# CarloSaccardi/GAN-Leaks

Hardware: AMD Instinct MI355X
Metric: attack query-images/sec (10k queries x 100k samples) + AUROC delta vs ref (higher is better)
Workload: dtype split-f16 (hi+lo, f32 accumulate; generator) + i8->i32 exact (distance)

## Files before the change

### gan-leaks_amd/csrc/gl_conv.h

```cpp
#pragma once
#include "gl_common.h"

struct GlGatherConv {
    const float *in;
    unsigned in_bytes;
    int64_t positions;
    int H, W, Cin;
    int up;
    const float *wpack;
    int cols;
    int cols_pad;
    int ntaps;
    uint32_t tap_dy[4], tap_dx[4];
    float *out;
    int Ho, Wo, omul;
    int oy[4], ox[4];
    int planar;
    int64_t ld_planar;
    int out_mode;
    int *sat_flag;
    const float *scale, *shift;
    int cmod;
    int act;
    const float *residual;
    const float *zero;
    const void *tail_w;
    float *tail_out;
    int64_t tail_ld;
    float tail_scale;
    float pixnorm_act;
    const float *rgb_w, *rgb_b;
    float *rgb_out;
    int rgb_n;
    float rgb_inv_act;
    char *tap_V;
    const float *tap_coef;
    int64_t tap_ldv, tap_off;
    int64_t tap_row0;
    int tap_fmt;
    char *tap_pool;
    float tap_scale, tap_eps;
};

static inline bool gl_vrow_blocked(int64_t K1_halves) { return K1_halves * 2 >= (2ll << 20); }
static inline int64_t gl_vrow_capacity(int64_t n, int64_t K1_halves) { return gl_vrow_blocked(K1_halves) ? (n + 255) / 256 * 256 : n; }

#if defined(__HIPCC__)
__device__ __forceinline__ char *gl_vrow_elem(char *V, int64_t ldv, int64_t row, int64_t k)
{
    if (ldv >= 0) return V + row * ldv + k * 2;
    return V + ((row >> 8) * (-ldv) + (k >> 6)) * 32768 + (row & 255) * 128 + (k & 63) * 2;
}

__device__ __forceinline__ float gl_tap_value(float v, float inv, float coef)
{
    float x = v * inv;
    asm volatile("" : "+v"(x));
    float t = x * coef;
    asm volatile("" : "+v"(t));
    return t;
}
#endif

void gl_pack_tail_weights_host(const float *w48xC, int channels, float scale, void *out);

static inline int64_t gl_conv_k_index(int tap, int ci, int ntaps) { return ((int64_t)(ci / 32) * ntaps + tap) * 32 + (ci % 32); }

int gl_launch_gather_conv(gl_ctx *ctx, const GlGatherConv &p, int phases);

int gl_launch_gather_conv_h3(gl_ctx *ctx, const GlGatherConv &p, int phases);
int gl_conv_h3_tile_channels(const GlGatherConv &p, int phases);
bool gl_conv_h3_tap_fusable(const GlGatherConv &p, int phases);
bool gl_conv_halo_applies(const GlGatherConv &p, int phases);
int gl_launch_conv_halo_h3(gl_ctx *ctx, const GlGatherConv &p);
int gl_launch_split_rows(gl_ctx *ctx, const float *in, int64_t n, int d, int dpad, float scale, void *out);
void gl_split_weights_host(const float *w, size_t rows, size_t K, float scale, void *out);

int gl_launch_col2im_rgb_tanh(gl_ctx *ctx, const float *P, int64_t ldp, int64_t n_img, int H, int W, const float *bias, float *out_f32,
                              uint8_t *out_u8);
```

### gan-leaks_amd/csrc/gl_conv_h3.hip

```cpp
#include "gl_conv.h"
#include "gl_conv_h3_epi.h"
#include <cstdlib>
#include <type_traits>

namespace {

using gl_h3::v8h;
using gl_h3::v4h;
using gl_h3::v4f;

constexpr int HBK_BYTES = 128;

template <int WC, int WP, int TC = 4, int TP = 4, bool FUSE_TAIL = false, bool UP = false, bool T4 = false>
__global__ void __launch_bounds__(64 * WC * WP, 2) gather_conv_h3_kernel(const GlGatherConv p, int m_tiles, int n_tiles, int phases)
{
#if __HIP_DEVICE_COMPILE__
    constexpr int HTC = 16 * TC * WC, HTP = 16 * TP * WP;
    constexpr int W_BYTES = HTC * HBK_BYTES, X_BYTES = HTP * HBK_BYTES, BUF = W_BYTES + X_BYTES;
    constexpr int NW = WC * WP;
    constexpr int PW = (HTC / 8) / NW, PX = (HTP / 8) / NW;
    static_assert(!T4 || (HTP == 256 && TP == 4 && WP == 4 && PX == 4 && !UP && !FUSE_TAIL), "T4: the 256-position tile with 4 position-waves of 4 fragments");
    extern __shared__ __attribute__((aligned(16))) char smem[];

    const unsigned inner = (unsigned)phases * (unsigned)n_tiles;
    const unsigned id = gl_xcd_remap(blockIdx.x, (unsigned)m_tiles * inner);
    const int mt = (int)(id / inner);
    const int phase = (int)((id % inner) / (unsigned)n_tiles);
    const int nt = (int)(id % (unsigned)n_tiles);
    const int64_t m0 = (int64_t)mt * HTP;
    const int c0 = nt * HTC;

    const int tid0 = threadIdx.x, lane0 = tid0 & 63;
    const int wave = __builtin_amdgcn_readfirstlane(tid0 >> 6);
    const int wc = wave / WP, wp_ = wave % WP;

    const int K = p.ntaps * p.Cin;
    const int nk = K / 32;
    const int HW = p.H * p.W;
    const uint32_t tdy = p.tap_dy[phase], tdx = p.tap_dx[phase];
    const char *wbase = reinterpret_cast<const char *>(p.wpack) + (int64_t)phase * p.cols_pad * K * 4;

    const int rsub = lane0 >> 3, slot = lane0 & 7;
    constexpr int up = UP ? 1 : 0;
    const int Ws = p.W >> up, Hs = p.H >> up;
    constexpr unsigned kOOB = 0xC0000000u;
    const unsigned lead_bytes = (unsigned)(p.W + 1) * (unsigned)p.Cin * 4u;
    const __amdgpu_buffer_rsrc_t x_rsrc =
        __builtin_amdgcn_make_buffer_rsrc(const_cast<char *>(reinterpret_cast<const char *>(p.in)) - (up ? 0 : (int64_t)lead_bytes), 0,
                                          (int)(p.in_bytes + (up ? 0u : 2u * lead_bytes)), 0x00020000);
    const __amdgpu_buffer_rsrc_t w_rsrc = __builtin_amdgcn_make_buffer_rsrc(const_cast<char *>(wbase), 0, (int)((unsigned)p.cols_pad * (unsigned)K * 4u), 0x00020000);
    unsigned x_voff0 = kOOB, x_mask2[(PX + 1) / 2], w_voff0 = 0;
#pragma unroll
    for (int i = 0; i < (PX + 1) / 2; ++i) x_mask2[i] = 0;
    auto x_mask_of = [&](int i) -> unsigned { return (x_mask2[i >> 1] >> ((i & 1) * 16)) & 0xFFFFu; };
    int x_img[UP ? PX : 1], x_yx[UP ? PX : 1];
    {
        const int r = wave * PW * 8 + rsub;
        w_voff0 = ((unsigned)(c0 + r) * (unsigned)K) * 4u + (unsigned)(slot ^ rsub) * 16u;
    }
    const unsigned w_step = 8u * (unsigned)K * 4u, x_step = 8u * (unsigned)p.Cin * 4u;
    auto t4_pos = [](int r) -> int { const int f = r >> 4, wpp = f >> 2, j = f & 3; return (r & 15) * 16 + 4 * j + ((j + wpp) & 3); };
#pragma unroll
    for (int i = 0; i < PX; ++i) {
        const int r = (wave * PX + i) * 8 + rsub;
        const int chunk = slot ^ (r & 7);
        const int64_t pos = m0 + (T4 ? t4_pos(r) : r);
        if constexpr (UP) { x_img[i] = 0; x_yx[i] = 0; }
        if (pos < p.positions) {
            const int64_t img = pos / HW;
            const int rem = (int)(pos - img * HW);
            const int y = rem / p.W, x = rem - y * p.W;
            for (int t = 0; t < p.ntaps; ++t) {
                const int yy = y + (int)((tdy >> (2 * t)) & 3u) - 1, xx = x + (int)((tdx >> (2 * t)) & 3u) - 1;
                if ((yy >= 0) & (yy < p.H) & (xx >= 0) & (xx < p.W)) x_mask2[i >> 1] |= 1u << (t + (i & 1) * 16);
            }
            if (i == 0 || T4) { if (i == 0) x_voff0 = (unsigned)pos * (unsigned)p.Cin * 4u + (unsigned)chunk * 16u; }
            if constexpr (UP) { x_img[i] = (int)(img * Hs * Ws); x_yx[i] = y | (x << 16); }
        }
    }

    auto stage = [&](int kt, char *buf) {
        const int tap = kt % p.ntaps;
        const int cc = kt / p.ntaps;
        const int dy = (int)((tdy >> (2 * tap)) & 3u) - 1;
        const int dx = (int)((tdx >> (2 * tap)) & 3u) - 1;
        const unsigned tapbit = 1u << tap;
#pragma unroll
        for (int i = 0; i < PW; ++i)
            __builtin_amdgcn_raw_ptr_buffer_load_lds(w_rsrc, (gl_lptr)(buf + (wave * PW + i) * 1024), 16, w_voff0, (unsigned)kt * 128u + (unsigned)i * w_step, 0, 0);
        if (!up) {
            const unsigned soff = (unsigned)(((dy + 1) * p.W + (dx + 1)) * p.Cin) * 4u + (unsigned)cc * 128u;
#pragma unroll
            for (int i = 0; i < PX; ++i) {
                const unsigned voff = (x_mask_of(i) & tapbit) ? x_voff0 : kOOB;
                unsigned piece = (unsigned)i * x_step;
                if constexpr (T4) piece = (unsigned)(t4_pos((wave * PX + i) * 8) - t4_pos(wave * PX * 8)) * (unsigned)p.Cin * 4u;
                __builtin_amdgcn_raw_ptr_buffer_load_lds(x_rsrc, (gl_lptr)(buf + W_BYTES + (wave * PX + i) * 1024), 16, voff, soff + piece, 0, 0);
            }
        } else {
            const unsigned soff = (unsigned)cc * 128u;
#pragma unroll
            for (int i = 0; i < PX; ++i) {
                const int r = (wave * PX + i) * 8 + rsub;
                const int yy = (x_yx[UP ? i : 0] & 0xFFFF) + dy, xx = (x_yx[UP ? i : 0] >> 16) + dx;
                const unsigned pix = (unsigned)(x_img[UP ? i : 0] + (yy >> 1) * Ws + (xx >> 1));
                const unsigned voff = (x_mask_of(i) & tapbit) ? pix * (unsigned)p.Cin * 4u + (unsigned)((slot ^ (r & 7)) * 16) : kOOB;
                __builtin_amdgcn_raw_ptr_buffer_load_lds(x_rsrc, (gl_lptr)(buf + W_BYTES + (wave * PX + i) * 1024), 16, voff, soff, 0, 0);
            }
        }
    };

    v4f acc[TC][TP];
#pragma unroll
    for (int i = 0; i < TC; ++i)
#pragma unroll
        for (int j = 0; j < TP; ++j) acc[i][j] = (v4f){0.f, 0.f, 0.f, 0.f};

    const int frow0 = lane0 & 15, fk0 = lane0 >> 4;
    auto compute = [&](const char *cur, int kt) {
        const char *lw = cur + (wc * 16 * TC) * HBK_BYTES;
        const char *lx = cur + W_BYTES + (wp_ * 16 * TP) * HBK_BYTES;
        v8h w_hi[TC], w_lo[TC], x_hi[TP], x_lo[TP];
        unsigned skip = 0;
        if constexpr (T4) {
            const int tap = kt % p.ntaps;
            const int dy = (int)((tdy >> (2 * tap)) & 3u) - 1, dx = (int)((tdx >> (2 * tap)) & 3u) - 1;
#pragma unroll
            for (int j = 0; j < TP; ++j) {
                const int yy = j + dy, xx = ((j + wp_) & 3) + dx;
                skip |= ((yy < 0) | (yy > 3) | (xx < 0) | (xx > 3)) ? 1u << j : 0u;
            }
        }
#pragma unroll
        for (int i = 0; i < TC; ++i) {
            const int r = i * 16 + frow0;
            w_hi[i] = *reinterpret_cast<const v8h *>(lw + r * HBK_BYTES + ((fk0 ^ (r & 7)) << 4));
            w_lo[i] = *reinterpret_cast<const v8h *>(lw + r * HBK_BYTES + (((4 + fk0) ^ (r & 7)) << 4));
        }
#pragma unroll
        for (int j = 0; j < TP; ++j) {
            const int r = j * 16 + frow0;
            x_hi[j] = *reinterpret_cast<const v8h *>(lx + r * HBK_BYTES + ((fk0 ^ (r & 7)) << 4));
            x_lo[j] = *reinterpret_cast<const v8h *>(lx + r * HBK_BYTES + (((4 + fk0) ^ (r & 7)) << 4));
        }
        if constexpr (T4) {
#pragma unroll
            for (int j = 0; j < TP; ++j) {
                if ((skip >> j) & 1u) continue;
#pragma unroll
                for (int i = 0; i < TC; ++i) {
                    acc[i][j] = __builtin_amdgcn_mfma_f32_16x16x32_f16(w_lo[i], x_hi[j], acc[i][j], 0, 0, 0);
                    acc[i][j] = __builtin_amdgcn_mfma_f32_16x16x32_f16(w_hi[i], x_lo[j], acc[i][j], 0, 0, 0);
                    acc[i][j] = __builtin_amdgcn_mfma_f32_16x16x32_f16(w_hi[i], x_hi[j], acc[i][j], 0, 0, 0);
                }
            }
        } else {
#pragma unroll
            for (int i = 0; i < TC; ++i)
#pragma unroll
                for (int j = 0; j < TP; ++j) {
                    acc[i][j] = __builtin_amdgcn_mfma_f32_16x16x32_f16(w_lo[i], x_hi[j], acc[i][j], 0, 0, 0);
                    acc[i][j] = __builtin_amdgcn_mfma_f32_16x16x32_f16(w_hi[i], x_lo[j], acc[i][j], 0, 0, 0);
                    acc[i][j] = __builtin_amdgcn_mfma_f32_16x16x32_f16(w_hi[i], x_hi[j], acc[i][j], 0, 0, 0);
                }
        }
    };
    stage(0, smem);
    for (int kt = 0; kt < nk; ++kt) {
        __syncthreads();
        if (kt + 1 < nk) stage(kt + 1, smem + ((kt + 1) & 1) * BUF);
        compute(smem + (kt & 1) * BUF, kt);
    }

    __syncthreads();
    int tid_again = threadIdx.x;
    asm volatile("" : "+v"(tid_again));
    const int tid = tid_again, lane = tid_again & 63, frow = tid_again & 15, fk = (tid_again & 63) >> 4;
    int *orow = reinterpret_cast<int *>(smem);
    if (tid < HTP) {
        const int64_t pos = m0 + (T4 ? t4_pos(tid) : tid);
        int o = -1;
        if (pos < p.positions) {
            const int64_t img = pos / HW;
            const int rem = (int)(pos - img * HW);
            const int y = rem / p.W, x = rem - y * p.W;
            o = (int)((img * p.Ho + (y * p.omul + p.oy[phase])) * p.Wo + (x * p.omul + p.ox[phase]));
        }
        orow[tid] = o;
    }
    __syncthreads();
    int o4[TP];
#pragma unroll
    for (int j = 0; j < TP; ++j) o4[j] = orow[wp_ * 16 * TP + j * 16 + frow];
    const float relu_floor = p.act == 1 ? 0.0f : -__builtin_inff();
    const float neg_slope = p.act == 2 ? 0.2f : 1.0f;
    bool saturated = false;
    if constexpr (FUSE_TAIL) {
        static_assert((WC == 2 || WC == 1) && TC == 4 && TP == 4, "fused tail: waves of 64 channels x 64 positions, 64 or 128 channels in all");
        v8h b_hi[2][TP], b_lo[2][TP];
#pragma unroll
        for (int i = 0; i < TC; ++i) {
            const int ch = wc * 64 + i * 16 + 4 * fk;
            float sc[4], sh[4];
#pragma unroll
            for (int r = 0; r < 4; ++r) { sc[r] = p.scale[ch + r]; sh[r] = p.shift[ch + r]; }
#pragma unroll
            for (int j = 0; j < TP; ++j)
#pragma unroll
                for (int r = 0; r < 4; ++r) {
                    float t = fmaf(acc[i][j][r], sc[r], sh[r]);
                    t = fmaxf(fmaxf(t, t * neg_slope), relu_floor);
                    const float c = fminf(fmaxf(t, -65504.0f), 65504.0f);
                    saturated |= (c != t) && (o4[j] >= 0);
                    const _Float16 h = (_Float16)c;
                    b_hi[i >> 1][j][(i & 1) * 4 + r] = h;
                    b_lo[i >> 1][j][(i & 1) * 4 + r] = (_Float16)(c - (float)h);
                }
        }
        v4f pacc[3][TP];
#pragma unroll
        for (int pt = 0; pt < 3; ++pt)
#pragma unroll
            for (int j = 0; j < TP; ++j) pacc[pt][j] = (v4f){0.f, 0.f, 0.f, 0.f};
        const v8h *tw = reinterpret_cast<const v8h *>(p.tail_w) + (size_t)wc * 3 * 2 * 2 * 64;
#pragma unroll
        for (int pt = 0; pt < 3; ++pt)
#pragma unroll
            for (int s2 = 0; s2 < 2; ++s2) {
                const v8h a_hi = tw[((pt * 2 + s2) * 2 + 0) * 64 + frow * 4 + fk];
                const v8h a_lo = tw[((pt * 2 + s2) * 2 + 1) * 64 + frow * 4 + fk];
#pragma unroll
                for (int j = 0; j < TP; ++j) {
                    pacc[pt][j] = __builtin_amdgcn_mfma_f32_16x16x32_f16(a_lo, b_hi[s2][j], pacc[pt][j], 0, 0, 0);
                    pacc[pt][j] = __builtin_amdgcn_mfma_f32_16x16x32_f16(a_hi, b_lo[s2][j], pacc[pt][j], 0, 0, 0);
                    pacc[pt][j] = __builtin_amdgcn_mfma_f32_16x16x32_f16(a_hi, b_hi[s2][j], pacc[pt][j], 0, 0, 0);
                }
            }
        float *xch = reinterpret_cast<float *>(smem + 4096) + (size_t)wp_ * 3 * TP * 4 * 64;
        if (WC == 2 && wc == 1) {
#pragma unroll
            for (int pt = 0; pt < 3; ++pt)
#pragma unroll
                for (int j = 0; j < TP; ++j)
#pragma unroll
                    for (int r = 0; r < 4; ++r) xch[((pt * TP + j) * 4 + r) * 64 + lane] = pacc[pt][j][r];
        }
        if (WC == 2) __syncthreads();
        if (wc == 0) {
#pragma unroll
            for (int pt = 0; pt < 3; ++pt)
#pragma unroll
                for (int j = 0; j < TP; ++j) {
                    const int o = o4[j];
                    if (o < 0) continue;
#pragma unroll
                    for (int r = 0; r < 4; ++r) {
                        const float v = pacc[pt][j][r] + (WC == 2 ? xch[((pt * TP + j) * 4 + r) * 64 + lane] : 0.0f);
                        p.tail_out[(int64_t)(pt * 16 + 4 * fk + r) * p.tail_ld + o] = v * p.tail_scale;
                    }
                }
        }
    } else {
        saturated |= gl_h3::epilogue<WC, WP, TC, TP>(p, acc, c0, wc, wp_, lane, o4, smem, p.tap_V ? (p.Wo >> 4) : 0);
    }
    if (__any(saturated) && lane == 0) atomicAdd(p.sat_flag, 1);
#endif
}

__global__ void __launch_bounds__(256) split_rows_kernel(const float *__restrict__ in, int64_t n, int d, int dpad, float scale, char *__restrict__ out)
{
    const int64_t i = (int64_t)blockIdx.x * blockDim.x + threadIdx.x;
    if (i >= n * dpad) return;
    const int64_t r = i / dpad;
    const int c = (int)(i - r * dpad);
    const float v = c < d ? fminf(fmaxf(in[r * d + c] * scale, -65504.0f), 65504.0f) : 0.0f;
    const _Float16 hi = (_Float16)v;
    const _Float16 lo = (_Float16)(v - (float)hi);
    char *dst = out + (r * dpad + (c >> 5) * 32) * 4 + (c & 31) * 2;
    *reinterpret_cast<_Float16 *>(dst) = hi;
    *reinterpret_cast<_Float16 *>(dst + 64) = lo;
}

}

template <int WC, int WP, int TC = 4, int TP = 4, bool FUSE_TAIL = false, bool UP = false, bool T4 = false>
static int launch_h3(gl_ctx *ctx, const GlGatherConv &p, int phases)
{
    if constexpr (!UP && !FUSE_TAIL && !T4) {
        if (p.up) return launch_h3<WC, WP, TC, TP, FUSE_TAIL, true>(ctx, p, phases);
    }
    if constexpr (WC == 2 && WP == 4 && TC == 8 && TP == 4 && !UP && !FUSE_TAIL && !T4) {
        const bool plain = !p.up && !p.tail_w && !p.tap_V && !p.rgb_out && p.pixnorm_act == 0.0f && !p.planar;
        if (plain && p.H == 4 && p.W == 4 && gl_tuning_int("GL_H3_T4", 1)) return launch_h3<WC, WP, TC, TP, false, false, true>(ctx, p, phases);
    }
    constexpr int HTC = 16 * TC * WC, HTP = 16 * TP * WP;
    const int64_t m_tiles = gl_ceil_div(p.positions, HTP);
    const int n_tiles = (int)gl_ceil_div(p.cols, HTC);
    GL_REQUIRE(m_tiles * n_tiles * phases < (1ll << 31), "gather_conv_h3: grid too large");
    constexpr int lds = 2 * (HTC + HTP) * HBK_BYTES;
    auto kern = gather_conv_h3_kernel<WC, WP, TC, TP, FUSE_TAIL, UP, T4>;
    GL_ONCE_PER_DEVICE(ctx, \
        GL_HIP(hipFuncSetAttribute(reinterpret_cast<const void *>(kern), hipFuncAttributeMaxDynamicSharedMemorySize, lds)););
    gl_prof_scope prof_(ctx, GL_PROF_GATHER_CONV);
    hipLaunchKernelGGL(kern, dim3((unsigned)(m_tiles * n_tiles * phases)), dim3(64 * WC * WP), lds, ctx->stream, p, (int)m_tiles, n_tiles, phases);
    GL_LAUNCH_CHECK();
    return GL_OK;
}

static int h3_tile_choice(const GlGatherConv &p, int phases)
{
    if (p.tail_w) return p.cols == 128 ? 3 : 4;
    if (p.cols <= 64) return 1;
    if (p.cols % 256 == 0 && gl_ceil_div(p.positions, 256) * (p.cols / 256) * phases >= 256) return 2;
    const int wide128 = gl_tuning_int("GL_H3_TILE128", 1);
    if (wide128 && p.cols <= 128 && gl_ceil_div(p.positions, 512) * phases >= 512) return 5;
    return 0;
}

int gl_conv_h3_tile_channels(const GlGatherConv &p, int phases)
{
    if (gl_conv_halo_applies(p, phases)) return p.cols <= 64 ? 64 : 128;
    const int t = h3_tile_choice(p, phases);
    return (t == 2 || t == 5) ? 0 : (t == 1 || t == 4) ? 64 : 128;
}

bool gl_conv_h3_tap_fusable(const GlGatherConv &p, int phases)
{
    const int enabled = gl_tuning_int("GL_TAP_FUSE", 1);
    if (!enabled || phases != 1 || p.tail_w || p.out_mode != 2 || p.omul != 1 || p.Ho != p.H || p.Wo != p.W || p.planar) return false;
    if (p.cols > gl_conv_h3_tile_channels(p, phases) || p.H % 2 != 0 || p.W % 16 != 0) return false;
    if (gl_conv_halo_applies(p, phases)) return true;
    return (p.W == 16 || p.W == 32) && p.positions % 64 == 0;
}

int gl_launch_gather_conv_h3(gl_ctx *ctx, const GlGatherConv &p_in, int phases)
{
    gl_make_current(ctx);
    GlGatherConv p = p_in;
    p.sat_flag = ctx->h3_sat;
    GL_REQUIRE(p.Cin % 32 == 0, "gather_conv_h3: Cin=%d must be a multiple of 32", p.Cin);
    GL_REQUIRE(p.cmod > 0 && p.cmod % 4 == 0, "gather_conv_h3: cmod=%d must be a positive multiple of 4", p.cmod);
    GL_REQUIRE(p.cols_pad % 128 == 0 && p.cols <= p.cols_pad && p.cols % 4 == 0, "gather_conv_h3: cols=%d / cols_pad=%d (multiple of 128)", p.cols, p.cols_pad);
    GL_REQUIRE(phases >= 1 && phases <= 4 && p.ntaps >= 1 && p.ntaps <= 16, "gather_conv_h3: bad phases/taps");
    GL_REQUIRE(p.act >= 0 && p.act <= 2 && !p.residual, "gather_conv_h3: activation %d / residual not supported", p.act);
    GL_REQUIRE(p.out_mode != 2 || p.cols % 32 == 0, "gather_conv_h3: split output needs cols %% 32 == 0");
    GL_REQUIRE(p.up == 0 || (p.up == 1 && p.H % 2 == 0 && p.W % 2 == 0), "gather_conv_h3: up must be 0 or 1");
    {
        const uint64_t imgs = (uint64_t)(p.positions / ((int64_t)p.H * p.W));
        const uint64_t bytes = imgs * (uint64_t)(p.H >> p.up) * (uint64_t)(p.W >> p.up) * (uint64_t)p.Cin * 4ull;
        GL_REQUIRE(bytes + 2ull * (uint64_t)(p.W + 1) * p.Cin * 4ull < 0xC0000000ull, "gather_conv_h3: input of %llu bytes exceeds 3 GiB; use a smaller pass",
                   (unsigned long long)bytes);
        p.in_bytes = (unsigned)bytes;
    }
    GL_REQUIRE((uint64_t)p.cols_pad * p.ntaps * p.Cin * 4ull < 0xC0000000ull, "gather_conv_h3: packed weights too large");
    if (p.positions == 0) return GL_OK;
    GL_REQUIRE(p.positions < (1ll << 31) && (p.positions / ((int64_t)p.H * p.W)) * p.Ho * p.Wo < (1ll << 31), "gather_conv_h3: too many positions");
    GL_REQUIRE(p.pixnorm_act == 0.0f || (p.out_mode == 2 && !p.tail_w && phases == 1 && p.cols <= gl_conv_h3_tile_channels(p, phases)),
               "gather_conv_h3: the fused PixelNorm needs split output and all %d channels in one tile", p.cols);
    GL_REQUIRE(!p.tap_V || (p.pixnorm_act == 0.0f && p.tap_coef && gl_conv_h3_tap_fusable(p, phases)), "gather_conv_h3: this layer's tap cannot be fused");
    if (p.tail_w)
        GL_REQUIRE(p.up == 0 && (p.cols == 128 || p.cols == 64) && p.cmod == p.cols && p.tail_out && p.tail_ld > 0, "gather_conv_h3: the fused tail needs a 64- or 128-channel layer");
    if (gl_conv_halo_applies(p, phases)) return gl_launch_conv_halo_h3(ctx, p);
    switch (h3_tile_choice(p, phases)) {
    case 3: return launch_h3<2, 2, 4, 4, true>(ctx, p, phases);
    case 4: return launch_h3<1, 4, 4, 4, true>(ctx, p, phases);
    case 1: return launch_h3<1, 4>(ctx, p, phases);
    case 2: return launch_h3<2, 4, 8, 4>(ctx, p, phases);
    case 5: return launch_h3<1, 8, 8, 4>(ctx, p, phases);
    default: return launch_h3<2, 2>(ctx, p, phases);
    }
}

int gl_launch_split_rows(gl_ctx *ctx, const float *in, int64_t n, int d, int dpad, float scale, void *out)
{
    gl_make_current(ctx);
    if (n == 0) return GL_OK;
    GL_REQUIRE(dpad % 32 == 0 && d <= dpad, "split_rows: bad padding");
    hipLaunchKernelGGL(split_rows_kernel, dim3((unsigned)gl_ceil_div(n * dpad, 256)), dim3(256), 0, ctx->stream, in, n, d, dpad, scale, reinterpret_cast<char *>(out));
    GL_LAUNCH_CHECK();
    return GL_OK;
}

void gl_split_weights_host(const float *w, size_t rows, size_t K, float scale, void *out)
{
    char *o = reinterpret_cast<char *>(out);
    for (size_t r = 0; r < rows; ++r)
// ... 32 lines not shown
```

### gan-leaks_amd/csrc/gl_conv_h3_epi.h

```cpp
#pragma once
#include "gl_conv.h"
#include <type_traits>

namespace gl_h3 {

typedef _Float16 v8h __attribute__((ext_vector_type(8)));
typedef _Float16 v4h __attribute__((ext_vector_type(4)));
typedef float v4f __attribute__((ext_vector_type(4)));

template <int WC, int WP, int TC, int TP>
__device__ __forceinline__ bool epilogue(const GlGatherConv &p, v4f (&acc)[TC][TP], int c0, int wc, int wp_, int lane, const int (&o4)[TP], char *smem,
                                         int pool_dj = 0)
{
    const int frow = lane & 15, fk = lane >> 4;
    const float relu_floor = p.act == 1 ? 0.0f : -__builtin_inff();
    const float neg_slope = p.act == 2 ? 0.2f : 1.0f;
    bool saturated = false;
    constexpr bool kFusable = TC <= 4;
    const bool pixnorm = kFusable && p.pixnorm_act > 0.0f;
    const bool tap = kFusable && p.tap_V != nullptr;
    float pinv[TP];
#pragma unroll
    for (int j = 0; j < TP; ++j) pinv[j] = 1.0f;
    if constexpr (kFusable) if (pixnorm || tap) {
        float tss[TC][TP];
#pragma unroll
        for (int i = 0; i < TC; ++i) {
            const int ch = c0 + wc * 16 * TC + i * 16 + 4 * fk;
            const bool real = ch < p.cols;
            const int chm = ch < p.cmod ? ch : ch % p.cmod;
            float sc[4], sh[4];
#pragma unroll
            for (int r = 0; r < 4; ++r) { sc[r] = real ? p.scale[chm + r] : 0.0f; sh[r] = real ? p.shift[chm + r] : 0.0f; }
#pragma unroll
            for (int j = 0; j < TP; ++j) {
                float s1 = 0.0f;
#pragma unroll
                for (int r = 0; r < 4; ++r) {
                    float t = fmaf(acc[i][j][r], sc[r], sh[r]);
                    t = fmaxf(fmaxf(t, t * neg_slope), relu_floor);
                    const float c = fminf(fmaxf(t, -65504.0f), 65504.0f);
                    saturated |= (c != t) && (o4[j] >= 0);
                    const _Float16 h = (_Float16)c;
// ... 154 lines not shown
            }
            if constexpr (WC > 1) {
                static_assert(WC == 2, "fused toRGB: one or two waves along the channels");
                float *xr = reinterpret_cast<float *>(smem + 8192 + 16384);
                __syncthreads();
                if (wc == 1) {
#pragma unroll
                    for (int j = 0; j < TP; ++j)
#pragma unroll
                        for (int c = 0; c < 4; ++c) xr[((wp_ * TP + j) * 4 + c) * 64 + lane] = res[j][c];
                }
                __syncthreads();
                if (wc == 1) return saturated;
#pragma unroll
                for (int j = 0; j < TP; ++j)
#pragma unroll
                    for (int c = 0; c < 4; ++c) res[j][c] = __fadd_rn(res[j][c], xr[((wp_ * TP + j) * 4 + c) * 64 + lane]);
            }
#pragma unroll
            for (int j = 0; j < TP; ++j) {
                float out4[4];
#pragma unroll
                for (int c = 0; c < 4; ++c) {
                    float sacc = res[j][c];
                    sacc = __fadd_rn(sacc, __shfl_xor(sacc, 16, 64));
                    sacc = __fadd_rn(sacc, __shfl_xor(sacc, 32, 64));
                    out4[c] = c < p.rgb_n ? fmaf(sacc, p.rgb_inv_act, p.rgb_b[c]) : 0.0f;
                }
                if (fk == 0 && o4[j] >= 0) *reinterpret_cast<float4 *>(p.rgb_out + (int64_t)o4[j] * 4) = make_float4(out4[0], out4[1], out4[2], out4[3]);
            }
            return saturated;
        }
    }
#pragma unroll
    for (int i = 0; i < TC; ++i) {
        const int ch = c0 + wc * 16 * TC + i * 16 + 4 * fk;
        if (ch >= p.cols) continue;
        float sc[4] = {0.f, 0.f, 0.f, 0.f}, sh[4] = {0.f, 0.f, 0.f, 0.f};
        if (!pixnorm) {
            const int chm = ch < p.cmod ? ch : ch % p.cmod;
#pragma unroll
            for (int r = 0; r < 4; ++r) { sc[r] = p.scale[chm + r]; sh[r] = p.shift[chm + r]; }
        }
#pragma unroll
        for (int j = 0; j < TP; ++j) {
            const int o = o4[j];
            if (o < 0) continue;
            float v[4];
#pragma unroll
            for (int r = 0; r < 4; ++r) {
                if (pixnorm) {
                    v[r] = __fmul_rn(acc[i][j][r], pinv[j]);
                } else {
                    float t = fmaf(acc[i][j][r], sc[r], sh[r]);
                    v[r] = fmaxf(fmaxf(t, t * neg_slope), relu_floor);
                }
            }
            if (p.out_mode == 2) {
                char *dst = reinterpret_cast<char *>(p.out) + (int64_t)o * p.cols * 4 + (ch >> 5) * 128 + (ch & 31) * 2;
                v4h hi, lo;
#pragma unroll
                for (int r = 0; r < 4; ++r) {
                    const float c = fminf(fmaxf(v[r], -65504.0f), 65504.0f);
                    saturated |= (c != v[r]);
                    hi[r] = (_Float16)c;
                    lo[r] = pixnorm ? (_Float16)fmaf(acc[i][j][r], pinv[j], -(float)hi[r]) : (_Float16)__fsub_rn(c, (float)hi[r]);
// ... 16 lines not shown
```

### gan-leaks_amd/csrc/gl_conv_halo.hip

```cpp
#include "gl_conv.h"
#include "gl_conv_h3_epi.h"
#include <cstdlib>

namespace {

using gl_h3::v4f;
using gl_h3::v8h;

constexpr int BLK = 16;
constexpr int HALO = BLK + 2;
constexpr int HPIX = HALO * HALO;
constexpr int HPIECES = (HPIX + 7) / 8;
constexpr int HBYTES = HPIECES * 1024;
constexpr int halo_bytes(int nw, bool ring) { return ring ? ((HPIECES + nw - 1) / nw) * nw * 1024 : HBYTES; }

template <int WC, bool RING = false>
__global__ void __launch_bounds__(256 * WC, 2) halo_conv_h3_kernel(const GlGatherConv p, int blocks_x, int blocks_per_img, unsigned total_blocks, int diag)
{
#if __HIP_DEVICE_COMPILE__
    constexpr int TC = 4, TP = 4, WP = 4, NW = WC * WP;
    constexpr int HTC = 64 * WC;
    constexpr int W_BYTES = HTC * 128;
    constexpr int NHBUF = WC;
    constexpr int PH = (HPIECES + NW - 1) / NW;
    constexpr int PW = (HTC / 8) / NW;
    constexpr int HB = halo_bytes(NW, RING);
    extern __shared__ __attribute__((aligned(16))) char smem[];
    char *const wbuf = smem + NHBUF * HB;

    const unsigned id = gl_xcd_remap(blockIdx.x, total_blocks);
    const int img = (int)(id / (unsigned)blocks_per_img);
    const int brem = (int)(id % (unsigned)blocks_per_img);
    const int y0 = (brem / blocks_x) * BLK, x0 = (brem % blocks_x) * BLK;

    const int tid = threadIdx.x, lane = tid & 63;
    const int wave = __builtin_amdgcn_readfirstlane(tid >> 6);
    const int wc = wave / WP, wp_ = wave % WP;
    const int rsub = lane >> 3, slot = lane & 7;
    const int frow = lane & 15, fk = lane >> 4;

    const int K = 9 * p.Cin, nchunks = p.Cin / 32;
    const int up = p.up;
    const int Ws = p.W >> up, Hs = p.H >> up;
    constexpr unsigned kOOB = 0xC0000000u;
    const __amdgpu_buffer_rsrc_t x_rsrc = __builtin_amdgcn_make_buffer_rsrc(const_cast<char *>(reinterpret_cast<const char *>(p.in)), 0, (int)p.in_bytes, 0x00020000);
    const __amdgpu_buffer_rsrc_t w_rsrc =
        __builtin_amdgcn_make_buffer_rsrc(const_cast<char *>(reinterpret_cast<const char *>(p.wpack)), 0, (int)((unsigned)p.cols_pad * (unsigned)K * 4u), 0x00020000);

    unsigned h_voff[PH];
// ... 104 lines not shown
                } else if (NHBUF == 2 && (tap == 1 || tap == 2) && more) {
                    asm volatile("s_waitcnt vmcnt(%0)" ::"n"(PW + PH) : "memory");
                } else {
                    asm volatile("s_waitcnt vmcnt(%0)" ::"n"(PW) : "memory");
                }
                __builtin_amdgcn_s_barrier();
                __builtin_amdgcn_sched_barrier(0);
                const int s2 = slot == 0 ? 2 : slot - 1;
                if (kt + 2 < nk) stage_w(kt + 2, wbuf + s2 * W_BYTES);
                if (NHBUF == 2 && tap == 0 && more) stage_halo(cc + 1, smem + ((cc + 1) & 1) * HB);
                compute(hb, wbuf + slot * W_BYTES, (tap / 3 - 1) * HALO + (tap % 3 - 1));
                slot = slot == 2 ? 0 : slot + 1;
            }
            if (NHBUF == 1 && more) {
                __builtin_amdgcn_s_barrier();
                stage_halo(cc + 1, smem);
            }
        }
    }

    __syncthreads();
    int o4[TP];
#pragma unroll
    for (int j = 0; j < TP; ++j) o4[j] = (img * p.Ho + y0 + wp_ * 4 + j) * p.Wo + x0 + frow;
    if (diag & 4) {
        float keep = 0.0f;
#pragma unroll
        for (int i = 0; i < TC; ++i)
#pragma unroll
            for (int j = 0; j < TP; ++j) keep += acc[i][j][0] + acc[i][j][1] + acc[i][j][2] + acc[i][j][3];
        if (keep == 123.456f) atomicAdd(p.sat_flag, 1);
        return;
    }
    const bool saturated = gl_h3::epilogue<WC, WP, TC, TP>(p, acc, 0, wc, wp_, lane, o4, smem, 1);
    if (__any(saturated) && lane == 0) atomicAdd(p.sat_flag, 1);
#endif
}

template <int WC, bool RING = false>
int launch_halo(gl_ctx *ctx, const GlGatherConv &p)
{
    const int bx = p.W / BLK, by = p.H / BLK;
    const int64_t imgs = p.positions / ((int64_t)p.H * p.W);
    const int64_t total = imgs * bx * by;
    GL_REQUIRE(total < (1ll << 31), "halo_conv_h3: grid too large");
    constexpr int lds = WC * halo_bytes(4 * WC, RING) + (RING ? 3 : 2) * 64 * WC * 128;
    auto kern = halo_conv_h3_kernel<WC, RING>;
    GL_ONCE_PER_DEVICE(ctx, \
        GL_HIP(hipFuncSetAttribute(reinterpret_cast<const void *>(kern), hipFuncAttributeMaxDynamicSharedMemorySize, lds)););
    gl_prof_scope prof_(ctx, GL_PROF_GATHER_CONV);
    hipLaunchKernelGGL(kern, dim3((unsigned)total), dim3(256 * WC), lds, ctx->stream, p, bx, bx * by, (unsigned)total, gl_tuning_int("GL_HALO_DIAG", 0));
    GL_LAUNCH_CHECK();
    return GL_OK;
}

}

bool gl_conv_halo_applies(const GlGatherConv &p, int phases)
{
    const int enabled = gl_tuning_int("GL_H3_HALO", 1);
    if (!enabled || phases != 1 || p.ntaps != 9 || p.tail_w || p.cols > 128 || p.Cin % 32 != 0) return false;
    uint32_t dy = 0, dx = 0;
    for (int t = 0; t < 9; ++t) { dy |= (uint32_t)(t / 3) << (2 * t); dx |= (uint32_t)(t % 3) << (2 * t); }
    if (p.tap_dy[0] != dy || p.tap_dx[0] != dx) return false;
    if (p.omul != 1 || p.Ho != p.H || p.Wo != p.W || p.oy[0] != 0 || p.ox[0] != 0 || p.planar || p.residual) return false;
    if (p.H % BLK != 0 || p.W % BLK != 0 || p.H < 32 || p.W < 32) return false;
    return p.positions / 256 >= 1024;
}

int gl_launch_conv_halo_h3(gl_ctx *ctx, const GlGatherConv &p)
{
#ifdef GL_TUNING
    if (gl_tuning_int("GL_HALO_RING", 0)) return p.cols <= 64 ? launch_halo<1, true>(ctx, p) : launch_halo<2, true>(ctx, p);
#endif
    return p.cols <= 64 ? launch_halo<1>(ctx, p) : launch_halo<2>(ctx, p);
}
```

Before: 51850.

## Trim per-tile overhead in gather conv with magic division and lean epilogues

Adds a LEAN path, on by default, to the gather and halo conv kernels. It replaces 64-bit divisions with precomputed magic-multiply division, builds border tap masks from per-phase class bitmasks instead of looping over taps, and steps tap and channel counters incrementally. It also issues the first weight stage before the mask setup and specializes the activation in the fused tail and split-store epilogue, with a fallback to the general path on overflow. The split-f16 epilogue now writes hi and lo pairs with permlane16 swaps into wide stores. It also adds tuning-only timestamp instrumentation, at the cost of more template variants and code size.

New measurement: 52310, median of 5. Within noise of the previous version (+0.9%).

```diff
diff --git a/gan-leaks_amd/csrc/gl_conv.h b/gan-leaks_amd/csrc/gl_conv.h
--- a/gan-leaks_amd/csrc/gl_conv.h
+++ b/gan-leaks_amd/csrc/gl_conv.h
@@ -1,5 +1,18 @@
 #pragma once
 #include "gl_common.h"
+
+struct GlDiv {
+    uint32_t mul;
+    uint32_t shift;
+};
+static inline GlDiv gl_div_make(uint32_t d)
+{
+    int l = 0;
+    while ((1ull << l) < d) ++l;
+    if ((1ull << l) == d) return GlDiv{0u, (uint32_t)l};
+    const uint64_t two = 1ull << (31 + l);
+    return GlDiv{(uint32_t)((two + d - 1) / d), (uint32_t)(l - 1)};
+}
 
 struct GlGatherConv {
     const float *in;
@@ -12,6 +25,8 @@
     int cols_pad;
     int ntaps;
     uint32_t tap_dy[4], tap_dx[4];
+    GlDiv div_hw, div_w;
+    uint64_t tap_cls[4];
     float *out;
     int Ho, Wo, omul;
     int oy[4], ox[4];
@@ -40,12 +55,17 @@
     int tap_fmt;
     char *tap_pool;
     float tap_scale, tap_eps;
+#ifdef GL_TUNING
+    unsigned long long *stamps;
+#endif
 };
 
 static inline bool gl_vrow_blocked(int64_t K1_halves) { return K1_halves * 2 >= (2ll << 20); }
 static inline int64_t gl_vrow_capacity(int64_t n, int64_t K1_halves) { return gl_vrow_blocked(K1_halves) ? (n + 255) / 256 * 256 : n; }
 
 #if defined(__HIPCC__)
+__device__ __forceinline__ unsigned gl_udiv(unsigned n, const GlDiv d) { return d.mul ? __umulhi(n, d.mul) >> d.shift : n >> d.shift; }
+
 __device__ __forceinline__ char *gl_vrow_elem(char *V, int64_t ldv, int64_t row, int64_t k)
 {
     if (ldv >= 0) return V + row * ldv + k * 2;
diff --git a/gan-leaks_amd/csrc/gl_conv_h3.hip b/gan-leaks_amd/csrc/gl_conv_h3.hip
--- a/gan-leaks_amd/csrc/gl_conv_h3.hip
+++ b/gan-leaks_amd/csrc/gl_conv_h3.hip
@@ -11,10 +11,26 @@
 
 constexpr int HBK_BYTES = 128;
 
-template <int WC, int WP, int TC = 4, int TP = 4, bool FUSE_TAIL = false, bool UP = false, bool T4 = false>
+template <int WC, int WP, int TC = 4, int TP = 4, bool FUSE_TAIL = false, bool UP = false, bool T4 = false, bool LEAN = true, bool STAMP = false>
 __global__ void __launch_bounds__(64 * WC * WP, 2) gather_conv_h3_kernel(const GlGatherConv p, int m_tiles, int n_tiles, int phases)
 {
 #if __HIP_DEVICE_COMPILE__
+#ifdef GL_TUNING
+    unsigned long long stamp[4] = {0, 0, 0, 0}, real[2] = {0, 0};
+#define GL_H3_STAMP(k)                                                                                   \
+    if constexpr (STAMP) {                                                                               \
+        __builtin_amdgcn_sched_barrier(0);                                                               \
+        asm volatile("s_memtime %0\n\ts_waitcnt lgkmcnt(0)" : "=s"(stamp[k])::"memory");                 \
+        __builtin_amdgcn_sched_barrier(0);                                                               \
+    }
+#else
+    static_assert(!STAMP, "stamps exist in the tuning build only");
+#define GL_H3_STAMP(k)
+#endif
+    GL_H3_STAMP(0)
+#ifdef GL_TUNING
+    if constexpr (STAMP) asm volatile("s_memrealtime %0\n\ts_waitcnt lgkmcnt(0)" : "=s"(real[0])::"memory");
+#endif
     constexpr int HTC = 16 * TC * WC, HTP = 16 * TP * WP;
     constexpr int W_BYTES = HTC * HBK_BYTES, X_BYTES = HTP * HBK_BYTES, BUF = W_BYTES + X_BYTES;
     constexpr int NW = WC * WP;
@@ -59,6 +75,13 @@
         w_voff0 = ((unsigned)(c0 + r) * (unsigned)K) * 4u + (unsigned)(slot ^ rsub) * 16u;
     }
     const unsigned w_step = 8u * (unsigned)K * 4u, x_step = 8u * (unsigned)p.Cin * 4u;
+    auto stage_w = [&](int kt, char *buf) {
+#pragma unroll
+        for (int i = 0; i < PW; ++i)
+            __builtin_amdgcn_raw_ptr_buffer_load_lds(w_rsrc, (gl_lptr)(buf + (wave * PW + i) * 1024), 16, w_voff0, (unsigned)kt * 128u + (unsigned)i * w_step, 0, 0);
+    };
+    if constexpr (LEAN) stage_w(0, smem);
+    const uint64_t tcls = p.tap_cls[phase];
     auto t4_pos = [](int r) -> int { const int f = r >> 4, wpp = f >> 2, j = f & 3; return (r & 15) * 16 + 4 * j + ((j + wpp) & 3); };
 #pragma unroll
     for (int i = 0; i < PX; ++i) {
@@ -67,27 +90,42 @@
         const int64_t pos = m0 + (T4 ? t4_pos(r) : r);
         if constexpr (UP) { x_img[i] = 0; x_yx[i] = 0; }
         if (pos < p.positions) {
-            const int64_t img = pos / HW;
-            const int rem = (int)(pos - img * HW);
-            const int y = rem / p.W, x = rem - y * p.W;
-            for (int t = 0; t < p.ntaps; ++t) {
-                const int yy = y + (int)((tdy >> (2 * t)) & 3u) - 1, xx = x + (int)((tdx >> (2 * t)) & 3u) - 1;
-                if ((yy >= 0) & (yy < p.H) & (xx >= 0) & (xx < p.W)) x_mask2[i >> 1] |= 1u << (t + (i & 1) * 16);
+            int64_t img;
+            int y, x;
+            if constexpr (LEAN) {
+                const unsigned im = gl_udiv((unsigned)pos, p.div_hw), rem = (unsigned)pos - im * (unsigned)HW;
+                img = im;
+                y = (int)gl_udiv(rem, p.div_w);
+                x = (int)rem - y * p.W;
+                const unsigned outside = (y == 0 ? (unsigned)tcls : 0u) | (y == p.H - 1 ? (unsigned)(tcls >> 16) : 0u) |
+                                         (x == 0 ? (unsigned)(tcls >> 32) : 0u) | (x == p.W - 1 ? (unsigned)(tcls >> 48) : 0u);
+                x_mask2[i >> 1] |= (((1u << p.ntaps) - 1u) & ~outside & 0xFFFFu) << ((i & 1) * 16);
+            } else {
+                img = pos / HW;
+                const int rem = (int)(pos - img * HW);
+                y = rem / p.W, x = rem - y * p.W;
+                for (int t = 0; t < p.ntaps; ++t) {
+                    const int yy = y + (int)((tdy >> (2 * t)) & 3u) - 1, xx = x + (int)((tdx >> (2 * t)) & 3u) - 1;
+                    if ((yy >= 0) & (yy < p.H) & (xx >= 0) & (xx < p.W)) x_mask2[i >> 1] |= 1u << (t + (i & 1) * 16);
+                }
             }
             if (i == 0 || T4) { if (i == 0) x_voff0 = (unsigned)pos * (unsigned)p.Cin * 4u + (unsigned)chunk * 16u; }
             if constexpr (UP) { x_img[i] = (int)(img * Hs * Ws); x_yx[i] = y | (x << 16); }
         }
     }
 
-    auto stage = [&](int kt, char *buf) {
-        const int tap = kt % p.ntaps;
-        const int cc = kt / p.ntaps;
+    int s_tap = 0, s_cc = 0, c_tap = 0;
+    auto stage_x = [&](int kt, char *buf) {
+        int tap, cc;
+        if constexpr (LEAN) {
+            tap = s_tap; cc = s_cc;
+            if (++s_tap == p.ntaps) { s_tap = 0; ++s_cc; }
+        } else {
+            tap = kt % p.ntaps; cc = kt / p.ntaps;
+        }
         const int dy = (int)((tdy >> (2 * tap)) & 3u) - 1;
         const int dx = (int)((tdx >> (2 * tap)) & 3u) - 1;
         const unsigned tapbit = 1u << tap;
-#pragma unroll
-        for (int i = 0; i < PW; ++i)
-            __builtin_amdgcn_raw_ptr_buffer_load_lds(w_rsrc, (gl_lptr)(buf + (wave * PW + i) * 1024), 16, w_voff0, (unsigned)kt * 128u + (unsigned)i * w_step, 0, 0);
         if (!up) {
             const unsigned soff = (unsigned)(((dy + 1) * p.W + (dx + 1)) * p.Cin) * 4u + (unsigned)cc * 128u;
 #pragma unroll
@@ -109,6 +147,7 @@
             }
         }
     };
+    auto stage = [&](int kt, char *buf) { stage_w(kt, buf); stage_x(kt, buf); };
 
     v4f acc[TC][TP];
 #pragma unroll
@@ -123,7 +162,9 @@
         v8h w_hi[TC], w_lo[TC], x_hi[TP], x_lo[TP];
         unsigned skip = 0;
         if constexpr (T4) {
-            const int tap = kt % p.ntaps;
+            int tap;
+            if constexpr (LEAN) { tap = c_tap; c_tap = c_tap + 1 == p.ntaps ? 0 : c_tap + 1; }
+            else tap = kt % p.ntaps;
             const int dy = (int)((tdy >> (2 * tap)) & 3u) - 1, dx = (int)((tdx >> (2 * tap)) & 3u) - 1;
 #pragma unroll
             for (int j = 0; j < TP; ++j) {
@@ -165,13 +206,16 @@
                 }
         }
     };
-    stage(0, smem);
+    if constexpr (LEAN) stage_x(0, smem);
+    else stage(0, smem);
     for (int kt = 0; kt < nk; ++kt) {
         __syncthreads();
+        if constexpr (STAMP) { if (kt == 0) { GL_H3_STAMP(1) } }
         if (kt + 1 < nk) stage(kt + 1, smem + ((kt + 1) & 1) * BUF);
         compute(smem + (kt & 1) * BUF, kt);
     }
 
+    GL_H3_STAMP(2)
     __syncthreads();
     int tid_again = threadIdx.x;
     asm volatile("" : "+v"(tid_again));
@@ -181,10 +225,16 @@
         const int64_t pos = m0 + (T4 ? t4_pos(tid) : tid);
         int o = -1;
         if (pos < p.positions) {
-            const int64_t img = pos / HW;
-            const int rem = (int)(pos - img * HW);
-            const int y = rem / p.W, x = rem - y * p.W;
-            o = (int)((img * p.Ho + (y * p.omul + p.oy[phase])) * p.Wo + (x * p.omul + p.ox[phase]));
+            if constexpr (LEAN) {
+                const unsigned img = gl_udiv((unsigned)pos, p.div_hw), rem = (unsigned)pos - img * (unsigned)HW;
+                const unsigned y = gl_udiv(rem, p.div_w), x = rem - y * (unsigned)p.W;
+                o = (int)((img * (unsigned)p.Ho + (y * (unsigned)p.omul + (unsigned)p.oy[phase])) * (unsigned)p.Wo + (x * (unsigned)p.omul + (unsigned)p.ox[phase]));
+            } else {
+                const int64_t img = pos / HW;
+                const int rem = (int)(pos - img * HW);
+                const int y = rem / p.W, x = rem - y * p.W;
+                o = (int)((img * p.Ho + (y * p.omul + p.oy[phase])) * p.Wo + (x * p.omul + p.ox[phase]));
+            }
         }
         orow[tid] = o;
     }
@@ -198,25 +248,44 @@
     if constexpr (FUSE_TAIL) {
         static_assert((WC == 2 || WC == 1) && TC == 4 && TP == 4, "fused tail: waves of 64 channels x 64 positions, 64 or 128 channels in all");
         v8h b_hi[2][TP], b_lo[2][TP];
-#pragma unroll
-        for (int i = 0; i < TC; ++i) {
-            const int ch = wc * 64 + i * 16 + 4 * fk;
-            float sc[4], sh[4];
-#pragma unroll
-            for (int r = 0; r < 4; ++r) { sc[r] = p.scale[ch + r]; sh[r] = p.shift[ch + r]; }
-#pragma unroll
-            for (int j = 0; j < TP; ++j)
-#pragma unroll
-                for (int r = 0; r < 4; ++r) {
-                    float t = fmaf(acc[i][j][r], sc[r], sh[r]);
-                    t = fmaxf(fmaxf(t, t * neg_slope), relu_floor);
-                    const float c = fminf(fmaxf(t, -65504.0f), 65504.0f);
-                    saturated |= (c != t) && (o4[j] >= 0);
-                    const _Float16 h = (_Float16)c;
-                    b_hi[i >> 1][j][(i & 1) * 4 + r] = h;
-                    b_lo[i >> 1][j][(i & 1) * 4 + r] = (_Float16)(c - (float)h);
-                }
-        }
+        auto activate = [&](auto act_c) -> bool {
+            constexpr int ACT = decltype(act_c)::value;
+            bool outside = false;
+#pragma unroll
+            for (int i = 0; i < TC; ++i) {
+                const int ch = wc * 64 + i * 16 + 4 * fk;
+                float sc[4], sh[4];
+#pragma unroll
+                for (int r = 0; r < 4; ++r) { sc[r] = p.scale[ch + r]; sh[r] = p.shift[ch + r]; }
+#pragma unroll
+                for (int j = 0; j < TP; ++j)
+#pragma unroll
+                    for (int r = 0; r < 4; ++r) {
+                        float t = fmaf(acc[i][j][r], sc[r], sh[r]);
+                        float c;
+                        if constexpr (ACT < 0) {
+                            t = fmaxf(fmaxf(t, t * neg_slope), relu_floor);
+                            c = fminf(fmaxf(t, -65504.0f), 65504.0f);
+                            saturated |= (c != t) && (o4[j] >= 0);
+                        } else {
+                            c = ACT == 1 ? fmaxf(t, 0.0f) : ACT == 2 ? fmaxf(t, t * 0.2f) : t;
+                            asm("" : "+v"(c));
+                            outside |= !(__builtin_fabsf(c) <= 65504.0f);
+                        }
+                        const _Float16 h = (_Float16)c;
+                        b_hi[i >> 1][j][(i & 1) * 4 + r] = h;
+                        b_lo[i >> 1][j][(i & 1) * 4 + r] = (_Float16)(c - (float)h);
+                    }
+            }
+            return outside;
+        };
+        bool general = true;
+        if constexpr (LEAN) {
+            const bool outside = p.act == 1 ? activate(std::integral_constant<int, 1>()) : p.act == 2 ? activate(std::integral_constant<int, 2>())
+                                                                                                         : activate(std::integral_constant<int, 0>());
+            general = __any(outside);
+        }
+        if (general) activate(std::integral_constant<int, -1>());
         v4f pacc[3][TP];
 #pragma unroll
         for (int pt = 0; pt < 3; ++pt)
@@ -247,6 +316,7 @@
         }
         if (WC == 2) __syncthreads();
         if (wc == 0) {
+            float *const col0 = p.tail_out + (int64_t)(4 * fk) * p.tail_ld;
 #pragma unroll
             for (int pt = 0; pt < 3; ++pt)
 #pragma unroll
@@ -256,13 +326,27 @@
 #pragma unroll
                     for (int r = 0; r < 4; ++r) {
                         const float v = pacc[pt][j][r] + (WC == 2 ? xch[((pt * TP + j) * 4 + r) * 64 + lane] : 0.0f);
-                        p.tail_out[(int64_t)(pt * 16 + 4 * fk + r) * p.tail_ld + o] = v * p.tail_scale;
+                        if constexpr (LEAN) col0[(int64_t)(pt * 16 + r) * p.tail_ld + o] = v * p.tail_scale;
+                        else p.tail_out[(int64_t)(pt * 16 + 4 * fk + r) * p.tail_ld + o] = v * p.tail_scale;
                     }
                 }
         }
     } else {
-        saturated |= gl_h3::epilogue<WC, WP, TC, TP>(p, acc, c0, wc, wp_, lane, o4, smem, p.tap_V ? (p.Wo >> 4) : 0);
-    }
+        saturated |= gl_h3::epilogue<WC, WP, TC, TP, LEAN>(p, acc, c0, wc, wp_, lane, o4, smem, p.tap_V ? (p.Wo >> 4) : 0);
+    }
+    GL_H3_STAMP(3)
+#ifdef GL_TUNING
+    if constexpr (STAMP) {
+        asm volatile("s_memrealtime %0\n\ts_waitcnt lgkmcnt(0)" : "=s"(real[1])::"memory");
+        if (tid == 0 && p.stamps) {
+#pragma unroll
+            for (int k = 0; k < 4; ++k) p.stamps[(size_t)blockIdx.x * 6 + k] = stamp[k];
+            p.stamps[(size_t)blockIdx.x * 6 + 4] = real[0];
+            p.stamps[(size_t)blockIdx.x * 6 + 5] = real[1];
+        }
+    }
+#endif
+#undef GL_H3_STAMP
     if (__any(saturated) && lane == 0) atomicAdd(p.sat_flag, 1);
 #endif
 }
@@ -283,22 +367,75 @@
 
 }
 
-template <int WC, int WP, int TC = 4, int TP = 4, bool FUSE_TAIL = false, bool UP = false, bool T4 = false>
-static int launch_h3(gl_ctx *ctx, const GlGatherConv &p, int phases)
-{
+#ifdef GL_TUNING
+static struct {
+    unsigned long long *buf;
+    int64_t cap, used;
+    std::vector<int64_t> log;
+} g_stamps;
+
+extern "C" int gl_tune_conv_stamps_begin(gl_ctx *ctx, void *buf, int64_t capacity_workgroups)
+{
+    GL_REQUIRE(ctx && buf && capacity_workgroups > 0, "gl_tune_conv_stamps_begin: bad argument");
+    g_stamps.buf = reinterpret_cast<unsigned long long *>(buf);
+    g_stamps.cap = capacity_workgroups;
+    g_stamps.used = 0;
+    g_stamps.log.clear();
+    return GL_OK;
+}
+
+extern "C" int gl_tune_conv_stamps_end(gl_ctx *ctx, int64_t *log_out, int max_launches, int *n_out)
+{
+    GL_REQUIRE(ctx && log_out && n_out && max_launches >= 0, "gl_tune_conv_stamps_end: bad argument");
+    g_stamps.buf = nullptr;
+    const int n = (int)(g_stamps.log.size() / 6);
+    for (int i = 0; i < n && i < max_launches; ++i)
+        for (int k = 0; k < 6; ++k) log_out[i * 6 + k] = g_stamps.log[(size_t)i * 6 + k];
+    *n_out = n;
+    return GL_OK;
+}
+#endif
+
+template <int WC, int WP, int TC = 4, int TP = 4, bool FUSE_TAIL = false, bool UP = false, bool T4 = false, bool LEAN = true, bool STAMP = false>
+static int launch_h3(gl_ctx *ctx, const GlGatherConv &p_in, int phases)
+{
+#ifdef GL_TUNING
+    if constexpr (LEAN) {
+        if (!gl_tuning_int("GL_H3_TILE_COST", 1)) return launch_h3<WC, WP, TC, TP, FUSE_TAIL, UP, T4, false, STAMP>(ctx, p_in, phases);
+    }
+#endif
     if constexpr (!UP && !FUSE_TAIL && !T4) {
-        if (p.up) return launch_h3<WC, WP, TC, TP, FUSE_TAIL, true>(ctx, p, phases);
+        if (p_in.up) return launch_h3<WC, WP, TC, TP, FUSE_TAIL, true, false, LEAN>(ctx, p_in, phases);
     }
     if constexpr (WC == 2 && WP == 4 && TC == 8 && TP == 4 && !UP && !FUSE_TAIL && !T4) {
-        const bool plain = !p.up && !p.tail_w && !p.tap_V && !p.rgb_out && p.pixnorm_act == 0.0f && !p.planar;
-        if (plain && p.H == 4 && p.W == 4 && gl_tuning_int("GL_H3_T4", 1)) return launch_h3<WC, WP, TC, TP, false, false, true>(ctx, p, phases);
+        const bool plain = !p_in.up && !p_in.tail_w && !p_in.tap_V && !p_in.rgb_out && p_in.pixnorm_act == 0.0f && !p_in.planar;
+        if (plain && p_in.H == 4 && p_in.W == 4 && gl_tuning_int("GL_H3_T4", 1)) return launch_h3<WC, WP, TC, TP, false, false, true, LEAN>(ctx, p_in, phases);
     }
     constexpr int HTC = 16 * TC * WC, HTP = 16 * TP * WP;
-    const int64_t m_tiles = gl_ceil_div(p.positions, HTP);
-    const int n_tiles = (int)gl_ceil_div(p.cols, HTC);
+    const int64_t m_tiles = gl_ceil_div(p_in.positions, HTP);
+    const int n_tiles = (int)gl_ceil_div(p_in.cols, HTC);
     GL_REQUIRE(m_tiles * n_tiles * phases < (1ll << 31), "gather_conv_h3: grid too large");
+#ifdef GL_TUNING
+    GlGatherConv p = p_in;
+    p.stamps = nullptr;
+    constexpr int kStampForm = (WC == 2 && WP == 4 && TC == 8 && !UP && !FUSE_TAIL) ? (T4 ? 0 : 1) : (WC == 2 && WP == 2 && FUSE_TAIL) ? 2 : -1;
+    if constexpr (kStampForm >= 0) {
+        const int64_t wgs = m_tiles * n_tiles * phases;
+        if constexpr (!STAMP) {
+            if (g_stamps.buf && g_stamps.used + wgs <= g_stamps.cap) return launch_h3<WC, WP, TC, TP, FUSE_TAIL, UP, T4, LEAN, true>(ctx, p_in, phases);
+        } else {
+            GL_REQUIRE(g_stamps.buf && g_stamps.used + wgs <= g_stamps.cap, "gather_conv_h3: stamp buffer too small");
+            p.stamps = g_stamps.buf + g_stamps.used * 6;
+            const int64_t entry[6] = {kStampForm, p.H, p.cols, wgs, g_stamps.used, LEAN ? 1 : 0};
+            g_stamps.log.insert(g_stamps.log.end(), entry, entry + 6);
+            g_stamps.used += wgs;
+        }
+    }
+#else
+    const GlGatherConv &p = p_in;
+#endif
     constexpr int lds = 2 * (HTC + HTP) * HBK_BYTES;
-    auto kern = gather_conv_h3_kernel<WC, WP, TC, TP, FUSE_TAIL, UP, T4>;
+    auto kern = gather_conv_h3_kernel<WC, WP, TC, TP, FUSE_TAIL, UP, T4, LEAN, STAMP>;
     GL_ONCE_PER_DEVICE(ctx, \
         GL_HIP(hipFuncSetAttribute(reinterpret_cast<const void *>(kern), hipFuncAttributeMaxDynamicSharedMemorySize, lds)););
     gl_prof_scope prof_(ctx, GL_PROF_GATHER_CONV);
@@ -352,6 +489,17 @@
                    (unsigned long long)bytes);
         p.in_bytes = (unsigned)bytes;
     }
+    p.div_hw = gl_div_make((uint32_t)(p.H * p.W));
+    p.div_w = gl_div_make((uint32_t)p.W);
+    for (int ph = 0; ph < phases; ++ph) {
+        uint64_t cls = 0;
+        for (int t = 0; t < p.ntaps; ++t) {
+            const uint32_t cy = (p.tap_dy[ph] >> (2 * t)) & 3u, cx = (p.tap_dx[ph] >> (2 * t)) & 3u;
+            GL_REQUIRE(cy <= 2 && cx <= 2, "gather_conv_h3: tap offsets must lie in -1..1");
+            cls |= (uint64_t)(cy == 0) << t | (uint64_t)(cy == 2) << (16 + t) | (uint64_t)(cx == 0) << (32 + t) | (uint64_t)(cx == 2) << (48 + t);
+        }
+        p.tap_cls[ph] = cls;
+    }
     GL_REQUIRE((uint64_t)p.cols_pad * p.ntaps * p.Cin * 4ull < 0xC0000000ull, "gather_conv_h3: packed weights too large");
     if (p.positions == 0) return GL_OK;
     GL_REQUIRE(p.positions < (1ll << 31) && (p.positions / ((int64_t)p.H * p.W)) * p.Ho * p.Wo < (1ll << 31), "gather_conv_h3: too many positions");
diff --git a/gan-leaks_amd/csrc/gl_conv_h3_epi.h b/gan-leaks_amd/csrc/gl_conv_h3_epi.h
--- a/gan-leaks_amd/csrc/gl_conv_h3_epi.h
+++ b/gan-leaks_amd/csrc/gl_conv_h3_epi.h
@@ -8,7 +8,7 @@
 typedef _Float16 v4h __attribute__((ext_vector_type(4)));
 typedef float v4f __attribute__((ext_vector_type(4)));
 
-template <int WC, int WP, int TC, int TP>
+template <int WC, int WP, int TC, int TP, bool LEAN = true>
 __device__ __forceinline__ bool epilogue(const GlGatherConv &p, v4f (&acc)[TC][TP], int c0, int wc, int wp_, int lane, const int (&o4)[TP], char *smem,
                                          int pool_dj = 0)
 {
@@ -229,6 +229,64 @@
             return saturated;
         }
     }
+    if constexpr (LEAN) if (p.out_mode == 2 && !pixnorm) {
+        static_assert(TC % 2 == 0, "split store: pairs of channel tiles");
+        typedef unsigned v4u __attribute__((ext_vector_type(4)));
+        char *row[TP];
+#pragma unroll
+        for (int j = 0; j < TP; ++j)
+            row[j] = reinterpret_cast<char *>(p.out) + ((int64_t)o4[j] * p.cols + (c0 + wc * 16 * TC)) * 4 + ((fk & 1) * 32 + (fk >> 1) * 16);
+        auto store_all = [&](auto act_c) -> bool {
+            constexpr int ACT = decltype(act_c)::value;
+            bool outside = false;
+#pragma unroll
+            for (int k = 0; k < TC / 2; ++k) {
+                if (c0 + wc * 16 * TC + 32 * k >= p.cols) continue;
+                float sc[2][4], sh[2][4];
+#pragma unroll
+                for (int h = 0; h < 2; ++h) {
+                    const int ch = c0 + wc * 16 * TC + (2 * k + h) * 16 + 4 * fk;
+                    const int chm = ch < p.cmod ? ch : ch % p.cmod;
+#pragma unroll
+                    for (int r = 0; r < 4; ++r) { sc[h][r] = p.scale[chm + r]; sh[h][r] = p.shift[chm + r]; }
+                }
+#pragma unroll
+                for (int j = 0; j < TP; ++j) {
+                    union { v4h h; unsigned u[2]; } hi[2], lo[2];
+#pragma unroll
+                    for (int h = 0; h < 2; ++h)
+#pragma unroll
+                        for (int r = 0; r < 4; ++r) {
+                            const float t = fmaf(acc[2 * k + h][j][r], sc[h][r], sh[h][r]);
+                            float v = ACT == 1 ? fmaxf(t, 0.0f) : ACT == 2 ? fmaxf(t, t * 0.2f) : t;
+                            asm("" : "+v"(v));
+                            outside |= !(__builtin_fabsf(v) <= 65504.0f);
+                            const _Float16 hh = (_Float16)v;
+                            hi[h].h[r] = hh;
+                            lo[h].h[r] = (_Float16)__fsub_rn(v, (float)hh);
+                        }
+                    v4u qh, ql;
+#pragma unroll
+                    for (int d = 0; d < 2; ++d) {
+                        const auto sh_ = __builtin_amdgcn_permlane16_swap(hi[0].u[d], hi[1].u[d], false, false);
+                        const auto sl_ = __builtin_amdgcn_permlane16_swap(lo[0].u[d], lo[1].u[d], false, false);
+                        qh[d] = sh_[0]; qh[2 + d] = sh_[1];
+                        ql[d] = sl_[0]; ql[2 + d] = sl_[1];
+                    }
+                    if (o4[j] >= 0) {
+                        *reinterpret_cast<v4u *>(row[j] + k * 128) = qh;
+                        *reinterpret_cast<v4u *>(row[j] + k * 128 + 64) = ql;
+                    }
+                }
+            }
+            return outside;
+        };
+        const bool outside = p.act == 1   ? store_all(std::integral_constant<int, 1>())
+                             : p.act == 2 ? store_all(std::integral_constant<int, 2>())
+                                          : store_all(std::integral_constant<int, 0>());
+        if (!__any(outside)) return saturated;
+        __builtin_amdgcn_fence(__ATOMIC_RELEASE, "agent");
+    }
 #pragma unroll
     for (int i = 0; i < TC; ++i) {
         const int ch = c0 + wc * 16 * TC + i * 16 + 4 * fk;
diff --git a/gan-leaks_amd/csrc/gl_conv_halo.hip b/gan-leaks_amd/csrc/gl_conv_halo.hip
--- a/gan-leaks_amd/csrc/gl_conv_halo.hip
+++ b/gan-leaks_amd/csrc/gl_conv_halo.hip
@@ -14,7 +14,7 @@
 constexpr int HBYTES = HPIECES * 1024;
 constexpr int halo_bytes(int nw, bool ring) { return ring ? ((HPIECES + nw - 1) / nw) * nw * 1024 : HBYTES; }
 
-template <int WC, bool RING = false>
+template <int WC, bool RING = false, bool LEAN = true>
 __global__ void __launch_bounds__(256 * WC, 2) halo_conv_h3_kernel(const GlGatherConv p, int blocks_x, int blocks_per_img, unsigned total_blocks, int diag)
 {
 #if __HIP_DEVICE_COMPILE__
@@ -185,20 +185,25 @@
         if (keep == 123.456f) atomicAdd(p.sat_flag, 1);
         return;
     }
-    const bool saturated = gl_h3::epilogue<WC, WP, TC, TP>(p, acc, 0, wc, wp_, lane, o4, smem, 1);
+    const bool saturated = gl_h3::epilogue<WC, WP, TC, TP, LEAN>(p, acc, 0, wc, wp_, lane, o4, smem, 1);
     if (__any(saturated) && lane == 0) atomicAdd(p.sat_flag, 1);
 #endif
 }
 
-template <int WC, bool RING = false>
+template <int WC, bool RING = false, bool LEAN = true>
 int launch_halo(gl_ctx *ctx, const GlGatherConv &p)
 {
+#ifdef GL_TUNING
+    if constexpr (LEAN) {
+        if (!gl_tuning_int("GL_H3_TILE_COST", 1)) return launch_halo<WC, RING, false>(ctx, p);
+    }
+#endif
     const int bx = p.W / BLK, by = p.H / BLK;
     const int64_t imgs = p.positions / ((int64_t)p.H * p.W);
     const int64_t total = imgs * bx * by;
     GL_REQUIRE(total < (1ll << 31), "halo_conv_h3: grid too large");
     constexpr int lds = WC * halo_bytes(4 * WC, RING) + (RING ? 3 : 2) * 64 * WC * 128;
-    auto kern = halo_conv_h3_kernel<WC, RING>;
+    auto kern = halo_conv_h3_kernel<WC, RING, LEAN>;
     GL_ONCE_PER_DEVICE(ctx, \
         GL_HIP(hipFuncSetAttribute(reinterpret_cast<const void *>(kern), hipFuncAttributeMaxDynamicSharedMemorySize, lds)););
     gl_prof_scope prof_(ctx, GL_PROF_GATHER_CONV);
```
